# ConsenSys/gnark-crypto

Measured on NVIDIA H100. Metric: bn254 G1 MultiExp scalar-muls/s, higher is better.
Workload: dtype u32

## Files before the change

### gnark-crypto_b200/csrc/curve.cuh

```cuda
#pragma once
#include "field.cuh"
#include "fp2.cuh"

namespace gmsm {

template <class F>
struct Affine {
  F x, y;
  GMSM_HD bool is_inf() const { return x.is_zero() && y.is_zero(); }
  GMSM_HD static Affine inf() { return Affine{F::zero(), F::zero()}; }
};

template <class F>
struct XYZZ {
  F x, y, zz, zzz;
  GMSM_HD bool is_inf() const { return zz.is_zero(); }
  GMSM_HD static XYZZ inf() { return XYZZ{F::zero(), F::zero(), F::zero(), F::zero()}; }
};

template <class F>
struct Jac {
  F x, y, z;
};

template <class F>
GMSM_HD XYZZ<F> xyzz_from_affine(const Affine<F>& a) {
  if (a.is_inf()) return XYZZ<F>::inf();
  return XYZZ<F>{a.x, a.y, F::one(), F::one()};
}

template <class F>
GMSM_HD XYZZ<F> xyzz_double_affine(const F& x, const F& y) {
  F U = f_dbl(y);
  F V = f_sqr(U);
  F W = f_mul(U, V);
  F S = f_mul(x, V);
  F XX = f_sqr(x);
  F M = f_add(f_dbl(XX), XX);
  F S2 = f_dbl(S);
#if defined(GMSM_DOT2)
  XYZZ<F> r;
  r.x = f_sub(f_sqr(M), S2);
  r.y = f_dot2(f_sub(S, r.x), M, W, f_neg(y));
#else
  F L = f_mul(W, y);
  XYZZ<F> r;
  r.x = f_sub(f_sqr(M), S2);
  r.y = f_sub(f_mul(f_sub(S, r.x), M), L);
#endif
  r.zz = V;
  r.zzz = W;
  return r;
}

template <class F>
GMSM_HD void xyzz_add_mixed(XYZZ<F>& p, const Affine<F>& a, bool negate) {
  if (a.is_inf()) return;
  F ay = negate ? f_neg(a.y) : a.y;
  if (p.zz.is_zero()) {
    p.x = a.x;
    p.y = ay;
    p.zz = F::one();
    p.zzz = F::one();
    return;
  }
  F P = f_sub(f_mul(a.x, p.zz), p.x);
  F R = f_sub(f_mul(ay, p.zzz), p.y);
  if (P.is_zero()) {
    if (R.is_zero()) {
      p = xyzz_double_affine(a.x, ay);
    } else {
      p.zz = F::zero();
      p.zzz = F::zero();
    }
    return;
  }
  F PP = f_sqr(P);
  F PPP = f_mul(P, PP);
  F Q = f_mul(p.x, PP);
  F RR = f_sqr(R);
  F X3 = f_sub(f_sub(RR, PPP), f_dbl(Q));
#if defined(GMSM_DOT2)
  F Y3 = f_dot2(f_sub(Q, X3), R, f_neg(p.y), PPP);
#else
  F Y3 = f_sub(f_mul(f_sub(Q, X3), R), f_mul(p.y, PPP));
#endif
  p.x = X3;
  p.y = Y3;
  p.zz = f_mul(p.zz, PP);
  p.zzz = f_mul(p.zzz, PPP);
}

template <class F>
GMSM_HD XYZZ<F> xyzz_double(const XYZZ<F>& q) {
  F U = f_dbl(q.y);
  F V = f_sqr(U);
  F W = f_mul(U, V);
  F S = f_mul(q.x, V);
  F XX = f_sqr(q.x);
  F M = f_add(f_dbl(XX), XX);
  F U2 = f_mul(W, q.y);
  XYZZ<F> r;
  r.x = f_sub(f_sub(f_sqr(M), S), S);
  r.y = f_sub(f_mul(f_sub(S, r.x), M), U2);
  r.zz = f_mul(V, q.zz);
  r.zzz = f_mul(W, q.zzz);
  return r;
}

template <class F>
GMSM_HD void xyzz_add(XYZZ<F>& p, const XYZZ<F>& q) {
  if (q.zz.is_zero()) return;
  if (p.zz.is_zero()) {
    p = q;
    return;
  }
  F U2 = f_mul(q.x, p.zz);
  F U1 = f_mul(p.x, q.zz);
  F S2 = f_mul(q.y, p.zzz);
  F S1 = f_mul(p.y, q.zzz);
  F P = f_sub(U2, U1);
  F R = f_sub(S2, S1);
  if (P.is_zero()) {
    if (R.is_zero()) {
      p = xyzz_double(q);
    } else {
      p.zz = F::zero();
      p.zzz = F::zero();
    }
    return;
  }
  F PP = f_sqr(P);
  F PPP = f_mul(P, PP);
  F Q = f_mul(U1, PP);
#if defined(GMSM_DOT2)
  F X3 = f_sub(f_sub(f_sub(f_sqr(R), PPP), Q), Q);
  F Y3 = f_dot2(f_sub(Q, X3), R, f_neg(S1), PPP);
#else
  F V = f_mul(S1, PPP);
  F X3 = f_sub(f_sub(f_sub(f_sqr(R), PPP), Q), Q);
  F Y3 = f_sub(f_mul(f_sub(Q, X3), R), V);
#endif
  p.x = X3;
  p.y = Y3;
  p.zz = f_mul(f_mul(p.zz, q.zz), PP);
  p.zzz = f_mul(f_mul(p.zzz, q.zzz), PPP);
}

template <class F>
GMSM_HD Jac<F> jac_double(const Jac<F>& p) {
  F A = f_sqr(p.x);
  F B = f_sqr(p.y);
  F C = f_sqr(B);
  F D = f_sub(f_sub(f_sqr(f_add(p.x, B)), A), C);
  D = f_dbl(D);
  F E = f_add(f_dbl(A), A);
  F Fq = f_sqr(E);
  Jac<F> r;
  r.z = f_dbl(f_mul(p.y, p.z));
  r.x = f_sub(Fq, f_dbl(D));
  F C8 = f_dbl(f_dbl(f_dbl(C)));
  r.y = f_sub(f_mul(E, f_sub(D, r.x)), C8);
  return r;
}

static constexpr int TAB_M = 8;
template <class F, class Ld, class St, class Dbl>
GMSM_HD void table_level_batch(int cnt, int c, Ld ld, St st, Dbl dbl) {
  Jac<F> pts[TAB_M];
  F pref[TAB_M];
  F prod = F::one();
  for (int i = 0; i < cnt; i++) {
    const Affine<F> a = ld(i);
    Jac<F> j = a.is_inf() ? Jac<F>{F::zero(), F::zero(), F::zero()} : Jac<F>{a.x, a.y, F::one()};
    for (int l = 0; l < c; l++) j = dbl(j);
    pts[i] = j;
    pref[i] = prod;
    if (!j.z.is_zero()) prod = f_mul(prod, j.z);
  }
  F inv = f_inv(prod);
  for (int i = cnt - 1; i >= 0; i--) {
    Affine<F> a = Affine<F>::inf();
    if (!pts[i].z.is_zero()) {
      const F zi = f_mul(inv, pref[i]);
      inv = f_mul(inv, pts[i].z);
      const F z2 = f_sqr(zi);
      a.x = f_mul(pts[i].x, z2);
      a.y = f_mul(f_mul(pts[i].y, z2), zi);
    }
    st(i, a);
  }
}

template <class F>
GMSM_HD XYZZ<F> jac_to_xyzz(const Jac<F>& p) {
  XYZZ<F> r;
  r.x = p.x;
  r.y = p.y;
  r.zz = f_sqr(p.z);
  r.zzz = f_mul(r.zz, p.z);
  return r;
}

template <class F>
GMSM_HD Jac<F> xyzz_to_jac(const XYZZ<F>& p) {
  if (p.zz.is_zero()) return Jac<F>{F::zero(), F::zero(), F::zero()};
  Jac<F> j;
  j.x = f_mul(f_sqr(p.zz), p.x);
  j.y = f_mul(f_sqr(p.zzz), p.y);
  j.z = p.zzz;
  return j;
}

template <class F>
GMSM_HD Affine<F> jac_to_affine(const Jac<F>& j) {
  if (j.z.is_zero()) return Affine<F>::inf();
  F a = f_inv(j.z);
  F b = f_sqr(a);
  Affine<F> r;
  r.x = f_mul(j.x, b);
  r.y = f_mul(f_mul(j.y, b), a);
  return r;
}

}
```

### gnark-crypto_b200/csrc/field.cuh

```cuda
#pragma once
#include <cstdint>

#include "field_consts.cuh"
#include "hd.cuh"

namespace gmsm {

#if defined(GMSM_EMULATE_PTX) && !defined(__CUDACC__)
static thread_local uint32_t emu_cf = 0;
GMSM_D uint32_t emu_add(uint32_t a, uint32_t b, uint32_t cin, bool set) {
  uint64_t s = (uint64_t)a + b + cin;
  if (set) emu_cf = (uint32_t)(s >> 32);
  return (uint32_t)s;
}
GMSM_D uint32_t emu_sub(uint32_t a, uint32_t b, uint32_t bin, bool set) {
  uint64_t d = (uint64_t)a - b - bin;
  if (set) emu_cf = (uint32_t)(d >> 32) & 1;
  return (uint32_t)d;
}
GMSM_D uint32_t add_cc(uint32_t a, uint32_t b) { return emu_add(a, b, 0, true); }
GMSM_D uint32_t addc_cc(uint32_t a, uint32_t b) { return emu_add(a, b, emu_cf, true); }
GMSM_D uint32_t addc(uint32_t a, uint32_t b) { return emu_add(a, b, emu_cf, false); }
GMSM_D uint32_t sub_cc(uint32_t a, uint32_t b) { return emu_sub(a, b, 0, true); }
GMSM_D uint32_t subc_cc(uint32_t a, uint32_t b) { return emu_sub(a, b, emu_cf, true); }
// ... 48 lines not shown
GMSM_D uint32_t madc_hi_cc(uint32_t a, uint32_t b, uint32_t c) {
  uint32_t r;
  asm volatile("madc.hi.cc.u32 %0, %1, %2, %3;" : "=r"(r) : "r"(a), "r"(b), "r"(c));
  return r;
}
GMSM_D uint32_t madc_hi(uint32_t a, uint32_t b, uint32_t c) {
  uint32_t r;
  asm volatile("madc.hi.u32 %0, %1, %2, %3;" : "=r"(r) : "r"(a), "r"(b), "r"(c));
  return r;
}
#endif

template <class P>
struct Fp {
  static constexpr int N = P::N;
  using Params = P;
  uint32_t l[N];

  GMSM_HD static Fp zero() {
    Fp r;
#pragma unroll
    for (int i = 0; i < N; i++) r.l[i] = 0;
    return r;
  }
  GMSM_HD static Fp one() {
    Fp r;
#pragma unroll
    for (int i = 0; i < N; i++) r.l[i] = P::one(i);
    return r;
  }
  GMSM_HD bool is_zero() const {
    uint32_t o = 0;
#pragma unroll
    for (int i = 0; i < N; i++) o |= l[i];
    return o == 0;
  }
  GMSM_HD bool operator==(const Fp& b) const {
    uint32_t o = 0;
#pragma unroll
    for (int i = 0; i < N; i++) o |= l[i] ^ b.l[i];
    return o == 0;
  }
  GMSM_HD bool operator!=(const Fp& b) const { return !(*this == b); }
};

template <class P>
GMSM_HD uint32_t invm() {
#if defined(__CUDA_ARCH__)
  if constexpr (P::MOD_IN_CONST_BANK) return P::mod_cb(P::N);
  else
#endif
  return P::INV;
}
template <class P>
GMSM_HD uint32_t modm(int j) {
#if defined(__CUDA_ARCH__)
  if constexpr (P::MOD_IN_CONST_BANK) return P::mod_cb(j);
  else
#endif
  return P::mod(j);
}

template <class P>
GMSM_HD void fp_reduce_once(Fp<P>& a, uint32_t carry = 0) {
  constexpr int N = P::N;
  uint32_t t[N];
#if defined(GMSM_PTX_PATH)
  t[0] = sub_cc(a.l[0], P::mod(0));
#pragma unroll
  for (int i = 1; i < N; i++) t[i] = subc_cc(a.l[i], P::mod(i));
  uint32_t borrow = subc(0, 0);
  if constexpr (P::FULL) borrow = carry ? 0u : borrow;
#pragma unroll
  for (int i = 0; i < N; i++) a.l[i] = borrow ? a.l[i] : t[i];
#else
  uint64_t br = 0;
  for (int i = 0; i < N; i++) {
    uint64_t d = (uint64_t)a.l[i] - P::mod(i) - br;
    t[i] = (uint32_t)d;
    br = (d >> 32) & 1;
  }
  if (!br || carry)
    for (int i = 0; i < N; i++) a.l[i] = t[i];
#endif
}

template <class P>
GMSM_HD Fp<P> fp_add(const Fp<P>& a, const Fp<P>& b) {
  constexpr int N = P::N;
  Fp<P> r;
#if defined(GMSM_PTX_PATH)
  uint32_t c = 0;
  r.l[0] = add_cc(a.l[0], b.l[0]);
#pragma unroll
  for (int i = 1; i < N - 1; i++) r.l[i] = addc_cc(a.l[i], b.l[i]);
  if constexpr (P::FULL) {
    r.l[N - 1] = addc_cc(a.l[N - 1], b.l[N - 1]);
    c = addc(0, 0);
  } else {
    r.l[N - 1] = addc(a.l[N - 1], b.l[N - 1]);
  }
#else
  uint64_t c = 0;
  for (int i = 0; i < N; i++) {
    c += (uint64_t)a.l[i] + b.l[i];
    r.l[i] = (uint32_t)c;
    c >>= 32;
  }
#endif
  fp_reduce_once(r, (uint32_t)c);
  return r;
}

template <class P>
GMSM_HD Fp<P> fp_dbl(const Fp<P>& a) {
  return fp_add(a, a);
}

template <class P>
GMSM_HD Fp<P> fp_sub(const Fp<P>& a, const Fp<P>& b) {
  constexpr int N = P::N;
  Fp<P> r;
#if defined(GMSM_PTX_PATH)
  r.l[0] = sub_cc(a.l[0], b.l[0]);
#pragma unroll
  for (int i = 1; i < N; i++) r.l[i] = subc_cc(a.l[i], b.l[i]);
  uint32_t mask = subc(0, 0);
  r.l[0] = add_cc(r.l[0], P::mod(0) & mask);
#pragma unroll
  for (int i = 1; i < N - 1; i++) r.l[i] = addc_cc(r.l[i], P::mod(i) & mask);
  r.l[N - 1] = addc(r.l[N - 1], P::mod(N - 1) & mask);
#else
  uint64_t br = 0;
  for (int i = 0; i < N; i++) {
    uint64_t d = (uint64_t)a.l[i] - b.l[i] - br;
    r.l[i] = (uint32_t)d;
    br = (d >> 32) & 1;
  }
  if (br) {
    uint64_t c = 0;
    for (int i = 0; i < N; i++) {
      c += (uint64_t)r.l[i] + P::mod(i);
      r.l[i] = (uint32_t)c;
      c >>= 32;
    }
  }
#endif
  return r;
}

template <class P>
GMSM_HD Fp<P> fp_neg(const Fp<P>& a) {
  return fp_sub(Fp<P>::zero(), a);
}

template <class P>
GMSM_HD Fp<P> fp_mul_cios(const Fp<P>& x, const Fp<P>& y) {
  constexpr int N = P::N;
  Fp<P> r;
  uint32_t t[N + 2];
#pragma unroll
  for (int i = 0; i < N + 2; i++) t[i] = 0;
#pragma unroll
  for (int i = 0; i < N; i++) {
    uint64_t c = 0;
#pragma unroll
    for (int j = 0; j < N; j++) {
      c += (uint64_t)x.l[j] * y.l[i] + t[j];
      t[j] = (uint32_t)c;
      c >>= 32;
    }
    c += t[N];
    t[N] = (uint32_t)c;
    t[N + 1] = (uint32_t)(c >> 32);
    uint32_t m = t[0] * P::INV;
    c = (uint64_t)m * P::mod(0) + t[0];
    c >>= 32;
#pragma unroll
    for (int j = 1; j < N; j++) {
      c += (uint64_t)m * P::mod(j) + t[j];
      t[j - 1] = (uint32_t)c;
      c >>= 32;
    }
    c += t[N];
    t[N - 1] = (uint32_t)c;
    t[N] = t[N + 1] + (uint32_t)(c >> 32);
  }
#pragma unroll
  for (int i = 0; i < N; i++) r.l[i] = t[i];
  fp_reduce_once(r, t[N]);
  return r;
}

template <class P>
GMSM_HD Fp<P> fp_mul_inline(const Fp<P>& x, const Fp<P>& y) {
  constexpr int N = P::N;
  Fp<P> r;
#if defined(GMSM_PTX_PATH) && !defined(GMSM_PORTABLE_MUL)
  uint32_t A[N + 2], B[N + 2];
#pragma unroll
  for (int i = 0; i < N + 2; i++) A[i] = B[i] = 0;
  uint32_t dprev = 0;
  uint32_t e0prev = 0;
#pragma unroll
  for (int i = 0; i < N; i++) {
    uint32_t* Ev = (i & 1) ? B : A;
    uint32_t* Od = (i & 1) ? A : B;
    const uint32_t bi = y.l[i];
    const uint32_t d = (i == 0) ? 0u : Od[1];
    if (i == 0) {
      Ev[0] = mad_lo_cc(x.l[0], bi, Ev[0]);
    } else {
      (void)add_cc(e0prev, dprev);
      Ev[0] = madc_lo_cc(x.l[0], bi, Ev[0]);
    }
    Ev[1] = madc_hi_cc(x.l[0], bi, Ev[1]);
#pragma unroll
    for (int j = 2; j < N; j += 2) {
      Ev[j] = madc_lo_cc(x.l[j], bi, Ev[j]);
      Ev[j + 1] = madc_hi_cc(x.l[j], bi, Ev[j + 1]);
    }
    if constexpr (P::FULL) Ev[N] = addc(Ev[N], 0);
    else Ev[N] = addc(0, 0);
    Od[0] = mad_lo_cc(x.l[1], bi, Od[2]);
    Od[1] = madc_hi_cc(x.l[1], bi, Od[3]);
#pragma unroll
    for (int j = 2; j < N; j += 2) {
      Od[j] = madc_lo_cc(x.l[j + 1], bi, Od[j + 2]);
      Od[j + 1] = madc_hi_cc(x.l[j + 1], bi, Od[j + 3]);
    }
    Od[N] = 0;
    const uint32_t m = (Ev[0] + d) * invm<P>();
    Ev[0] = mad_lo_cc(modm<P>(0), m, Ev[0]);
    Ev[1] = madc_hi_cc(modm<P>(0), m, Ev[1]);
#pragma unroll
    for (int j = 2; j < N; j += 2) {
      Ev[j] = madc_lo_cc(modm<P>(j), m, Ev[j]);
      Ev[j + 1] = madc_hi_cc(modm<P>(j), m, Ev[j + 1]);
    }
    Ev[N] = addc(Ev[N], 0);
    Od[0] = mad_lo_cc(modm<P>(1), m, Od[0]);
    Od[1] = madc_hi_cc(modm<P>(1), m, Od[1]);
#pragma unroll
    for (int j = 2; j < N; j += 2) {
      Od[j] = madc_lo_cc(modm<P>(j + 1), m, Od[j]);
      Od[j + 1] = madc_hi_cc(modm<P>(j + 1), m, Od[j + 1]);
    }
    if constexpr (P::FULL) Od[N] = addc(0, 0);
    e0prev = Ev[0];
    dprev = d;
  }
  (void)add_cc(e0prev, dprev);
  r.l[0] = addc_cc(A[0], B[1]);
#pragma unroll
  for (int i = 1; i < N - 1; i++) r.l[i] = addc_cc(A[i], B[i + 1]);
  if constexpr (P::FULL) {
    r.l[N - 1] = addc_cc(A[N - 1], B[N]);
    fp_reduce_once(r, addc(A[N], 0));
  } else {
    r.l[N - 1] = addc(A[N - 1], B[N]);
    fp_reduce_once(r);
  }
#else
  return fp_mul_cios(x, y);
#endif
  return r;
}

#if defined(__CUDA_ARCH__) && defined(GMSM_MUL_NOINLINE)
template <class P> GMSM_HD Fp<P> fp_mul_karatsuba(const Fp<P>& x, const Fp<P>& y);
template <class P>
__device__ __noinline__ Fp<P> fp_mul_ni(Fp<P> x, Fp<P> y) {
#if defined(GMSM_MUL_KARATSUBA)
  if constexpr (P::N % 4 == 0 && (P::mod(P::N - 1) >> 30) == 0) return fp_mul_karatsuba(x, y);
  else
#endif
  return fp_mul_inline(x, y);
}
template <class P>
GMSM_HD Fp<P> fp_mul(const Fp<P>& x, const Fp<P>& y) {
  return fp_mul_ni<P>(x, y);
}
#else
template <class P> GMSM_HD Fp<P> fp_mul_karatsuba(const Fp<P>& x, const Fp<P>& y);
template <class P>
GMSM_HD Fp<P> fp_mul(const Fp<P>& x, const Fp<P>& y) {
#if defined(GMSM_MUL_KARATSUBA)
  if constexpr (P::N % 4 == 0 && (P::mod(P::N - 1) >> 30) == 0) return fp_mul_karatsuba(x, y);
  else
#endif
  return fp_mul_inline(x, y);
}
#endif

#if defined(GMSM_SQR_DEDICATED) && defined(GMSM_PTX_PATH) && !defined(GMSM_PORTABLE_MUL)
template <class P>
GMSM_HD Fp<P> fp_sqr_inline(const Fp<P>& x) {
  constexpr int N = P::N;
  static_assert((P::mod(N - 1) >> 30) == 0, "needs two spare top bits (2x in N limbs, frames below 3q)");
  Fp<P> r;
  uint32_t x2[N];
  x2[0] = x.l[0] << 1;
#pragma unroll
  for (int j = 1; j < N; j++) x2[j] = (x.l[j] << 1) | (x.l[j - 1] >> 31);
  uint32_t A[N + 2], B[N + 2];
#pragma unroll
// ... 449 lines not shown
      Ev[j] = madc_lo_cc(modm<P>(j), m, Ev[j]);
      Ev[j + 1] = madc_hi_cc(modm<P>(j), m, Ev[j + 1]);
    }
    Ev[N] = addc(Ev[N], 0);
    Od[0] = mad_lo_cc(modm<P>(1), m, Od[0]);
    Od[1] = madc_hi_cc(modm<P>(1), m, Od[1]);
#pragma unroll
    for (int j = 2; j < N; j += 2) {
      Od[j] = madc_lo_cc(modm<P>(j + 1), m, Od[j]);
      Od[j + 1] = madc_hi_cc(modm<P>(j + 1), m, Od[j + 1]);
    }
    GMSM_NO_CARRY();
    e0prev = Ev[0];
    dprev = d;
  }
  (void)add_cc(e0prev, dprev);
  out[0] = addc_cc(A[0], B[1]);
#pragma unroll
  for (int i = 1; i < N - 1; i++) out[i] = addc_cc(A[i], B[i + 1]);
  out[N - 1] = addc(A[N - 1], B[N]);
#else
  uint32_t t[N + 2];
  for (int i = 0; i < N; i++) t[i] = v[i];
  t[N] = t[N + 1] = 0;
  for (int i = 0; i < N; i++) {
    const uint32_t m = t[0] * P::INV;
    uint64_t c = (uint64_t)m * P::mod(0) + t[0];
    c >>= 32;
    for (int j = 1; j < N; j++) {
      c += (uint64_t)m * P::mod(j) + t[j];
      t[j - 1] = (uint32_t)c;
      c >>= 32;
    }
    c += t[N];
    t[N - 1] = (uint32_t)c;
    t[N] = (uint32_t)(c >> 32);
  }
  for (int i = 0; i < N; i++) out[i] = t[i];
#endif
}

template <class P, int NRED = 3>
GMSM_HD Fp<P> fp_redc_wide(const uint32_t* t) {
  constexpr int N = P::N;
  uint32_t lo[N];
  fp_redc_half<P>(t, lo);
  Fp<P> r;
#if defined(GMSM_PTX_PATH)
  r.l[0] = add_cc(lo[0], t[N]);
#pragma unroll
  for (int i = 1; i < N - 1; i++) r.l[i] = addc_cc(lo[i], t[N + i]);
  r.l[N - 1] = addc(lo[N - 1], t[2 * N - 1]);
#else
  uint64_t c = 0;
  for (int i = 0; i < N; i++) {
    c += (uint64_t)lo[i] + t[N + i];
    r.l[i] = (uint32_t)c;
    c >>= 32;
  }
#endif
#pragma unroll
  for (int k = 0; k < NRED; k++) fp_reduce_once(r);
  return r;
}

template <class P>
GMSM_HD Fp<P> fp_mul_karatsuba(const Fp<P>& x, const Fp<P>& y) {
  uint32_t t[2 * P::N];
  mul_wide_karatsuba<P::N>(x.l, y.l, t);
  return fp_redc_wide<P, 1>(t);
}

template <class P>
GMSM_HD Fp<P> fp_mul_split(const Fp<P>& x, const Fp<P>& y) {
  uint32_t t[2 * P::N];
  fp_mul_wide<P>(x.l, y.l, t);
  return fp_redc_wide<P>(t);
}

template <class P>
GMSM_HD Fp<P> fp_from_mont(const Fp<P>& x) {
  Fp<P> o = Fp<P>::zero();
  o.l[0] = 1;
  return fp_mul(x, o);
}

template <class P>
GMSM_HD Fp<P> fp_to_mont(const Fp<P>& x) {
  Fp<P> r2;
#pragma unroll
  for (int i = 0; i < P::N; i++) r2.l[i] = P::r2(i);
  return fp_mul(x, r2);
}

template <class P>
GMSM_HD Fp<P> fp_inv_fermat(const Fp<P>& x) {
  constexpr int N = P::N;
  uint32_t e[N];
  {
    uint64_t br = 2;
    for (int i = 0; i < N; i++) {
      uint64_t d = (uint64_t)P::mod(i) - br;
      e[i] = (uint32_t)d;
      br = (d >> 32) & 1;
    }
  }
  Fp<P> acc = Fp<P>::one();
  bool started = false;
  for (int i = 32 * N - 1; i >= 0; i--) {
    if (started) acc = fp_sqr(acc);
    if ((e[i >> 5] >> (i & 31)) & 1) {
      acc = started ? fp_mul(acc, x) : x;
      started = true;
    }
  }
  return acc;
}

template <class P>
GMSM_HD Fp<P> fp_inv(const Fp<P>& x) {
  constexpr int N = P::N;
  if (x.is_zero()) return x;
  uint32_t u[N], v[N], x1[N], x2[N];
  for (int i = 0; i < N; i++) { u[i] = x.l[i]; v[i] = P::mod(i); x1[i] = 0; x2[i] = 0; }
  x1[0] = 1;
  auto is_one = [](const uint32_t* a) { uint32_t o = a[0] ^ 1u; for (int i = 1; i < N; i++) o |= a[i]; return o == 0; };
  auto shr1 = [](uint32_t* a, uint32_t top) { for (int i = 0; i < N - 1; i++) a[i] = (a[i] >> 1) | (a[i + 1] << 31); a[N - 1] = (a[N - 1] >> 1) | (top << 31); };
  auto add_mod = [](uint32_t* a) { uint64_t c = 0; for (int i = 0; i < N; i++) { c += (uint64_t)a[i] + P::mod(i); a[i] = (uint32_t)c; c >>= 32; } return (uint32_t)c; };
  auto geq = [](const uint32_t* a, const uint32_t* b) { for (int i = N - 1; i >= 0; i--) { if (a[i] != b[i]) return a[i] > b[i]; } return true; };
  auto sub = [](uint32_t* a, const uint32_t* b) { uint64_t br = 0; for (int i = 0; i < N; i++) { uint64_t d = (uint64_t)a[i] - b[i] - br; a[i] = (uint32_t)d; br = (d >> 32) & 1; } return (uint32_t)br; };
  auto halve = [&](uint32_t* w, uint32_t* y) {
    shr1(w, 0);
    const uint32_t top = (y[0] & 1u) ? add_mod(y) : 0u;
    shr1(y, top);
  };
  auto sub_mod = [&](uint32_t* a, const uint32_t* b) { if (sub(a, b)) add_mod(a); };
  while (!is_one(u) && !is_one(v)) {
    while (!(u[0] & 1u)) halve(u, x1);
    while (!(v[0] & 1u)) halve(v, x2);
    if (geq(u, v)) { sub(u, v); sub_mod(x1, x2); } else { sub(v, u); sub_mod(x2, x1); }
  }
  Fp<P> r, r2;
  for (int i = 0; i < N; i++) { r.l[i] = is_one(u) ? x1[i] : x2[i]; r2.l[i] = P::r2(i); }
  return fp_mul(fp_mul(r, r2), r2);
}

template <class P> GMSM_HD Fp<P> f_add(const Fp<P>& a, const Fp<P>& b) { return fp_add(a, b); }
template <class P> GMSM_HD Fp<P> f_sub(const Fp<P>& a, const Fp<P>& b) { return fp_sub(a, b); }
template <class P> GMSM_HD Fp<P> f_mul(const Fp<P>& a, const Fp<P>& b) { return fp_mul(a, b); }
template <class P> GMSM_HD Fp<P> f_sqr(const Fp<P>& a) { return fp_sqr(a); }
template <class P> GMSM_HD Fp<P> f_dot2(const Fp<P>& x, const Fp<P>& y, const Fp<P>& u, const Fp<P>& v) { return fp_dot2(x, y, u, v); }
template <class P> GMSM_HD Fp<P> f_dbl(const Fp<P>& a) { return fp_dbl(a); }
template <class P> GMSM_HD Fp<P> f_neg(const Fp<P>& a) { return fp_neg(a); }
template <class P> GMSM_HD Fp<P> f_inv(const Fp<P>& a) { return fp_inv(a); }

}
```

### gnark-crypto_b200/csrc/fp2.cuh

```cuda
#pragma once
#include "field.cuh"

namespace gmsm {

template <class P>
struct Fp2 {
  using Params = P;
  static constexpr int N = 2 * P::N;
  Fp<P> a0, a1;
  GMSM_HD static Fp2 zero() { return Fp2{Fp<P>::zero(), Fp<P>::zero()}; }
  GMSM_HD static Fp2 one() { return Fp2{Fp<P>::one(), Fp<P>::zero()}; }
  GMSM_HD bool is_zero() const { return a0.is_zero() && a1.is_zero(); }
  GMSM_HD bool operator==(const Fp2& b) const { return a0 == b.a0 && a1 == b.a1; }
  GMSM_HD bool operator!=(const Fp2& b) const { return !(*this == b); }
};

template <class P> GMSM_HD Fp2<P> f_add(const Fp2<P>& a, const Fp2<P>& b) { return Fp2<P>{fp_add(a.a0, b.a0), fp_add(a.a1, b.a1)}; }
template <class P> GMSM_HD Fp2<P> f_sub(const Fp2<P>& a, const Fp2<P>& b) { return Fp2<P>{fp_sub(a.a0, b.a0), fp_sub(a.a1, b.a1)}; }
template <class P> GMSM_HD Fp2<P> f_dbl(const Fp2<P>& a) { return Fp2<P>{fp_dbl(a.a0), fp_dbl(a.a1)}; }
template <class P> GMSM_HD Fp2<P> f_neg(const Fp2<P>& a) { return Fp2<P>{fp_neg(a.a0), fp_neg(a.a1)}; }

template <class P>
GMSM_HD Fp<P> fp_mul_by5(const Fp<P>& c) {
  return fp_add(fp_dbl(fp_dbl(c)), c);
}

#if defined(GMSM_FP2_LAZY)
template <class P>
GMSM_HD Fp2<P> fp2_mul_lazy_inline(const Fp2<P>& x, const Fp2<P>& y) {
    constexpr int N = P::N;
    uint32_t sx[N], sy[N], T0[2 * N], T1[2 * N], T2[2 * N];
#if defined(GMSM_PTX_PATH)
    sx[0] = add_cc(x.a0.l[0], x.a1.l[0]);
#pragma unroll
    for (int i = 1; i < N - 1; i++) sx[i] = addc_cc(x.a0.l[i], x.a1.l[i]);
    sx[N - 1] = addc(x.a0.l[N - 1], x.a1.l[N - 1]);
    sy[0] = add_cc(y.a0.l[0], y.a1.l[0]);
#pragma unroll
    for (int i = 1; i < N - 1; i++) sy[i] = addc_cc(y.a0.l[i], y.a1.l[i]);
    sy[N - 1] = addc(y.a0.l[N - 1], y.a1.l[N - 1]);
#else
    { uint64_t c = 0; for (int i = 0; i < N; i++) { c += (uint64_t)x.a0.l[i] + x.a1.l[i]; sx[i] = (uint32_t)c; c >>= 32; } }
    { uint64_t c = 0; for (int i = 0; i < N; i++) { c += (uint64_t)y.a0.l[i] + y.a1.l[i]; sy[i] = (uint32_t)c; c >>= 32; } }
#endif
    fp_mul_wide<P>(x.a0.l, y.a0.l, T0);
    fp_mul_wide<P>(x.a1.l, y.a1.l, T1);
    fp_mul_wide<P>(sx, sy, T2);
#if defined(GMSM_PTX_PATH)
    T2[0] = sub_cc(T2[0], T0[0]);
#pragma unroll
    for (int i = 1; i < 2 * N - 1; i++) T2[i] = subc_cc(T2[i], T0[i]);
    T2[2 * N - 1] = subc(T2[2 * N - 1], T0[2 * N - 1]);
    T2[0] = sub_cc(T2[0], T1[0]);
#pragma unroll
    for (int i = 1; i < 2 * N - 1; i++) T2[i] = subc_cc(T2[i], T1[i]);
    T2[2 * N - 1] = subc(T2[2 * N - 1], T1[2 * N - 1]);
    T0[0] = sub_cc(T0[0], T1[0]);
#pragma unroll
    for (int i = 1; i < 2 * N - 1; i++) T0[i] = subc_cc(T0[i], T1[i]);
    T0[2 * N - 1] = subc(T0[2 * N - 1], T1[2 * N - 1]);
    T0[N] = add_cc(T0[N], P::mod(0));
#pragma unroll
    for (int i = 1; i < N - 1; i++) T0[N + i] = addc_cc(T0[N + i], P::mod(i));
    T0[2 * N - 1] = addc(T0[2 * N - 1], P::mod(N - 1));
#else
    { uint64_t br = 0; for (int i = 0; i < 2 * N; i++) { uint64_t d = (uint64_t)T2[i] - T0[i] - br; T2[i] = (uint32_t)d; br = (d >> 32) & 1; } }
    { uint64_t br = 0; for (int i = 0; i < 2 * N; i++) { uint64_t d = (uint64_t)T2[i] - T1[i] - br; T2[i] = (uint32_t)d; br = (d >> 32) & 1; } }
    { uint64_t br = 0; for (int i = 0; i < 2 * N; i++) { uint64_t d = (uint64_t)T0[i] - T1[i] - br; T0[i] = (uint32_t)d; br = (d >> 32) & 1; } }
    { uint64_t c = 0; for (int i = 0; i < N; i++) { c += (uint64_t)T0[N + i] + P::mod(i); T0[N + i] = (uint32_t)c; c >>= 32; } }
#endif
    Fp2<P> z;
    z.a1 = fp_redc_wide<P, 1>(T2);
    z.a0 = fp_redc_wide<P, 2>(T0);
    return z;
}
#if defined(__CUDA_ARCH__) && defined(GMSM_MUL_NOINLINE)
template <class P>
__device__ __noinline__ Fp2<P> fp2_mul_lazy_ni(Fp2<P> x, Fp2<P> y) {
  return fp2_mul_lazy_inline(x, y);
}
#endif
#endif

template <class P>
GMSM_HD Fp2<P> f_mul(const Fp2<P>& x, const Fp2<P>& y) {
  static_assert(P::FP2_NONRES == -1 || P::FP2_NONRES == -5, "supported quadratic non-residues");
#if defined(GMSM_FP2_LAZY)
  if constexpr (P::FP2_NONRES == -1 && (P::mod(P::N - 1) >> 30) == 0) {
#if defined(__CUDA_ARCH__) && defined(GMSM_MUL_NOINLINE)
    return fp2_mul_lazy_ni<P>(x, y);
#else
    return fp2_mul_lazy_inline(x, y);
#endif
  }
#endif
#if defined(GMSM_FP2_DOT2) && defined(GMSM_DOT2)
  Fp2<P> z;
  const Fp<P> by1 = (P::FP2_NONRES == -5) ? fp_neg(fp_mul_by5(y.a1)) : fp_neg(y.a1);
  z.a0 = fp_dot2(x.a0, y.a0, x.a1, by1);
  z.a1 = fp_dot2(x.a0, y.a1, x.a1, y.a0);
  return z;
#else
  Fp<P> a = fp_add(x.a0, x.a1);
  Fp<P> b = fp_add(y.a0, y.a1);
  a = fp_mul(a, b);
  b = fp_mul(x.a0, y.a0);
  Fp<P> c = fp_mul(x.a1, y.a1);
  Fp2<P> z;
  z.a1 = fp_sub(fp_sub(a, b), c);
  if (P::FP2_NONRES == -5) c = fp_mul_by5(c);
  z.a0 = fp_sub(b, c);
  return z;
#endif
}

template <class P>
GMSM_HD Fp2<P> f_sqr(const Fp2<P>& x) {
  Fp<P> a = fp_add(x.a0, x.a1);
  Fp<P> b = (P::FP2_NONRES == -5) ? fp_sub(x.a0, fp_mul_by5(x.a1)) : fp_sub(x.a0, x.a1);
  a = fp_mul(a, b);
  b = fp_dbl(fp_mul(x.a0, x.a1));
  if (P::FP2_NONRES == -5) a = fp_add(a, fp_dbl(b));
  return Fp2<P>{a, b};
}

template <class P>
GMSM_HD Fp2<P> f_dot2(const Fp2<P>& x, const Fp2<P>& y, const Fp2<P>& u, const Fp2<P>& v) {
#if defined(GMSM_DOT4)
  const Fp<P> by1 = (P::FP2_NONRES == -5) ? fp_neg(fp_mul_by5(y.a1)) : fp_neg(y.a1);
  const Fp<P> bv1 = (P::FP2_NONRES == -5) ? fp_neg(fp_mul_by5(v.a1)) : fp_neg(v.a1);
  Fp2<P> z;
  z.a0 = fp_dot4(x.a0, y.a0, x.a1, by1, u.a0, v.a0, u.a1, bv1);
  z.a1 = fp_dot4(x.a0, y.a1, x.a1, y.a0, u.a0, v.a1, u.a1, v.a0);
  return z;
#else
  return f_add(f_mul(x, y), f_mul(u, v));
#endif
}

template <class P>
GMSM_HD Fp2<P> f_inv(const Fp2<P>& x) {
  Fp<P> t0 = fp_sqr(x.a0);
  Fp<P> t1 = fp_sqr(x.a1);
  if (P::FP2_NONRES == -5) t1 = fp_mul_by5(t1);
  t0 = fp_add(t0, t1);
  t1 = fp_inv(t0);
  return Fp2<P>{fp_mul(x.a0, t1), fp_neg(fp_mul(x.a1, t1))};
}

}
```

### gnark-crypto_b200/csrc/testops.cuh

```cuda
#pragma once
#include "groups.cuh"

namespace gmsm {

template <class T>
GMSM_HD T rd(const uint32_t* p) {
  T r;
  uint32_t* w = reinterpret_cast<uint32_t*>(&r);
  for (int i = 0; i < (int)(sizeof(T) / 4); i++) w[i] = p[i];
  return r;
}
template <class T>
GMSM_HD void wr(uint32_t* p, const T& r) {
  const uint32_t* w = reinterpret_cast<const uint32_t*>(&r);
  for (int i = 0; i < (int)(sizeof(T) / 4); i++) p[i] = w[i];
}

template <class G>
GMSM_HD void test_op_sizes(int op, int* wa, int* wb, int* wo) {
  constexpr int FW = G::F::N;
  switch (op) {
    case 0: case 1: case 2: *wa = FW; *wb = FW; *wo = FW; break;
    case 3: case 4: case 5: case 6: *wa = FW; *wb = 0; *wo = FW; break;
    case 7: case 8: *wa = 4 * FW; *wb = 2 * FW; *wo = 4 * FW; break;
    case 9: *wa = 4 * FW; *wb = 4 * FW; *wo = 4 * FW; break;
    case 10: *wa = 4 * FW; *wb = 0; *wo = 4 * FW; break;
    case 11: *wa = 4 * FW; *wb = 0; *wo = 2 * FW; break;
    case 12: *wa = G::Fr::N; *wb = 0; *wo = G::Fr::N; break;
    case 13: *wa = 2 * FW; *wb = 2 * FW; *wo = FW; break;
    default: *wa = *wb = *wo = 0;
  }
}

template <class G>
GMSM_HD void test_op_one(int op, const uint32_t* a, const uint32_t* b, uint32_t* o) {
  using F = typename G::F;
  switch (op) {
    case 0: wr(o, f_mul(rd<F>(a), rd<F>(b))); break;
    case 1: wr(o, f_add(rd<F>(a), rd<F>(b))); break;
    case 2: wr(o, f_sub(rd<F>(a), rd<F>(b))); break;
    case 3: wr(o, f_sqr(rd<F>(a))); break;
    case 4: wr(o, f_neg(rd<F>(a))); break;
    case 5: wr(o, f_dbl(rd<F>(a))); break;
    case 6: wr(o, f_inv(rd<F>(a))); break;
    case 7: case 8: {
      XYZZ<F> p = rd<XYZZ<F>>(a);
      xyzz_add_mixed(p, rd<Affine<F>>(b), op == 8);
      wr(o, p);
    } break;
    case 9: {
      XYZZ<F> p = rd<XYZZ<F>>(a);
      xyzz_add(p, rd<XYZZ<F>>(b));
      wr(o, p);
    } break;
    case 10: wr(o, xyzz_double(rd<XYZZ<F>>(a))); break;
    case 11: wr(o, jac_to_affine(xyzz_to_jac(rd<XYZZ<F>>(a)))); break;
    case 12: wr(o, fp_from_mont(rd<typename G::Fr>(a))); break;
    case 13: wr(o, f_dot2(rd<F>(a), rd<F>(b), rd<F>(a + G::F::N), rd<F>(b + G::F::N))); break;
    default: break;
  }
}


}
```

### include/gmsm.h

```cpp
#ifndef GMSM_H
#define GMSM_H

#include <stddef.h>
#include <stdint.h>

#ifdef __cplusplus
extern "C" {
#endif

typedef enum {
  GMSM_BN254_G1 = 0,
  GMSM_BN254_G2 = 1,
  GMSM_BLS12381_G1 = 2,
  GMSM_BLS12381_G2 = 3,
  GMSM_BLS12377_G1 = 4,
  GMSM_BLS12377_G2 = 5,
  GMSM_SECP256K1_G1 = 6,
  GMSM_BW6761_G1 = 7,
  GMSM_BW6761_G2 = 8,
  GMSM_BLS24315_G1 = 9,
  GMSM_BLS24317_G1 = 10,
  GMSM_BW6633_G1 = 11,
  GMSM_BW6633_G2 = 12
} gmsm_curve_t;

enum {
  GMSM_OK = 0,
  GMSM_EINVAL = 1,
  GMSM_ECUDA = 2,
  GMSM_ENOMEM = 3,
  GMSM_ENODEV = 4
};

const char* gmsm_last_error(void);
const char* gmsm_version(void);

size_t gmsm_affine_bytes(gmsm_curve_t curve);
size_t gmsm_scalar_bytes(gmsm_curve_t curve);
size_t gmsm_jac_bytes(gmsm_curve_t curve);
size_t gmsm_xyzz_bytes(gmsm_curve_t curve);

int gmsm_bn254_g1_multiexp(const uint64_t* points, const uint64_t* scalars, size_t n, int nb_tasks,
                           uint64_t out_jac[12]);
int gmsm_bn254_g2_multiexp(const uint64_t* points, const uint64_t* scalars, size_t n, int nb_tasks,
                           uint64_t out_jac[24]);
int gmsm_bls12381_g1_multiexp(const uint64_t* points, const uint64_t* scalars, size_t n, int nb_tasks,
                              uint64_t out_jac[18]);
int gmsm_bls12381_g2_multiexp(const uint64_t* points, const uint64_t* scalars, size_t n, int nb_tasks,
                              uint64_t out_jac[36]);
int gmsm_bls12377_g1_multiexp(const uint64_t* points, const uint64_t* scalars, size_t n, int nb_tasks,
                              uint64_t out_jac[18]);
int gmsm_bls12377_g2_multiexp(const uint64_t* points, const uint64_t* scalars, size_t n, int nb_tasks,
                              uint64_t out_jac[36]);
int gmsm_secp256k1_g1_multiexp(const uint64_t* points, const uint64_t* scalars, size_t n, int nb_tasks,
                               uint64_t out_jac[12]);
int gmsm_bw6761_g1_multiexp(const uint64_t* points, const uint64_t* scalars , size_t n, int nb_tasks,
                            uint64_t out_jac[36]);
int gmsm_bw6761_g2_multiexp(const uint64_t* points, const uint64_t* scalars , size_t n, int nb_tasks,
                            uint64_t out_jac[36]);
int gmsm_bls24315_g1_multiexp(const uint64_t* points, const uint64_t* scalars, size_t n, int nb_tasks,
                              uint64_t out_jac[15]);
int gmsm_bls24317_g1_multiexp(const uint64_t* points, const uint64_t* scalars, size_t n, int nb_tasks,
                              uint64_t out_jac[15]);
int gmsm_bw6633_g1_multiexp(const uint64_t* points, const uint64_t* scalars , size_t n, int nb_tasks,
                            uint64_t out_jac[30]);
int gmsm_bw6633_g2_multiexp(const uint64_t* points, const uint64_t* scalars , size_t n, int nb_tasks,
                            uint64_t out_jac[30]);
int gmsm_multiexp(gmsm_curve_t curve, const uint64_t* points, const uint64_t* scalars, size_t n,
                  int nb_tasks, uint64_t* out_jac);
int gmsm_choose_window_bits(gmsm_curve_t curve, size_t n_total);
int gmsm_multiexp_window_sums(gmsm_curve_t curve, const uint64_t* points, const uint64_t* scalars, size_t n, int c,
                              int device, void* out_partials);
int gmsm_last_oneshot_launches(void);

typedef struct gmsm_bases gmsm_bases_t;
gmsm_bases_t* gmsm_bases_upload(gmsm_curve_t curve, const uint64_t* points, size_t n, int device);
int gmsm_bases_multiexp(gmsm_bases_t* bases, size_t offset, const uint64_t* scalars, size_t n,
                        int nb_tasks, uint64_t* out_jac);
void gmsm_bases_free(gmsm_bases_t* bases);
int gmsm_bases_multiexp_device(gmsm_bases_t* bases, size_t offset, const void* d_scalars, size_t n, int nb_tasks,
                               uint64_t* out_jac, void* stream);
int gmsm_bases_precompute(gmsm_bases_t* bases, int c);
int gmsm_bases_table_bits(const gmsm_bases_t* bases);

typedef struct gmsm_ctx gmsm_ctx_t;
gmsm_ctx_t* gmsm_ctx_create(gmsm_curve_t curve, size_t max_n, int c, int device);
void gmsm_ctx_destroy(gmsm_ctx_t* ctx);
int gmsm_ctx_window_bits(const gmsm_ctx_t* ctx);
int gmsm_ctx_num_windows(const gmsm_ctx_t* ctx);
size_t gmsm_ctx_workspace_bytes(const gmsm_ctx_t* ctx);
int gmsm_ctx_last_launches(const gmsm_ctx_t* ctx);
int gmsm_ctx_msm_device(gmsm_ctx_t* ctx, const void* d_points, const void* d_scalars, size_t n,
                        void* d_out_jac, void* stream);
int gmsm_ctx_window_sums_device(gmsm_ctx_t* ctx, const void* d_points, const void* d_scalars, size_t n,
                                void* d_partials, void* stream);
int gmsm_ctx_finalize_device(gmsm_ctx_t* ctx, const void* d_partials, int nranks, void* d_out_jac,
                             void* stream);
gmsm_ctx_t* gmsm_ctx_create_tables(gmsm_curve_t curve, size_t max_n, int c, int device);
int gmsm_tables_build_device(gmsm_curve_t curve, int c, const void* d_points, size_t n, void* d_table,
                             size_t row_stride, void* stream);
int gmsm_ctx_msm_tables_device(gmsm_ctx_t* ctx, const void* d_table, size_t row_stride, size_t offset,
                               const void* d_scalars, size_t n, void* d_out_jac, void* stream);
void gmsm_ctx_set_profiling(gmsm_ctx_t* ctx, int on);
int gmsm_ctx_last_stage_ms(gmsm_ctx_t* ctx, float out_ms[8]);

int gmsm_generate_multiples_device(gmsm_curve_t curve, const uint64_t* base_affine_host, uint64_t start,
                                   size_t n, void* d_out_points, void* stream);

int gmsm_batch_scalar_mul(gmsm_curve_t curve, const uint64_t* base_affine, const uint64_t* scalars, size_t n,
                          uint64_t* out_points);

int gmsm_g1_decode(gmsm_curve_t curve, const uint8_t* bytes, size_t n, int raw, int check_on_curve, uint64_t* out_points);
int gmsm_g1_decode_device(gmsm_curve_t curve, const void* d_bytes, size_t n, int raw, int check_on_curve, void* d_points,
                          void* d_first_error, void* stream);

typedef struct gmsm_fft_domain gmsm_fft_domain_t;
enum {
  GMSM_FR_BN254 = 0, GMSM_FR_BLS12381 = 1, GMSM_FR_BLS12377 = 2,
  GMSM_FR_BLS24315 = 3,
  GMSM_FR_BLS24317 = 4,
  GMSM_FR_BW6633 = 5,
  GMSM_FR_BW6761 = 6
};
enum { GMSM_DIT = 0, GMSM_DIF = 1 };
size_t gmsm_fft_fr_bytes(int fr_field);
gmsm_fft_domain_t* gmsm_fft_domain_create(int fr_field, uint64_t m, const uint64_t* shift, int device);
void gmsm_fft_domain_free(gmsm_fft_domain_t* domain);
uint64_t gmsm_fft_domain_cardinality(const gmsm_fft_domain_t* domain);
int gmsm_fft_domain_constants(const gmsm_fft_domain_t* domain, uint64_t* out);
int gmsm_fft(gmsm_fft_domain_t* domain, uint64_t* a, size_t n, int decimation, int coset);
int gmsm_fft_inverse(gmsm_fft_domain_t* domain, uint64_t* a, size_t n, int decimation, int coset);
int gmsm_fft_device(gmsm_fft_domain_t* domain, void* d_a, size_t n, int inverse, int decimation, int coset, void* stream);
int gmsm_fft_bit_reverse_device(gmsm_fft_domain_t* domain, void* d_a, size_t n, void* stream);

size_t gmsm_fr_poly_workspace_bytes(int fr_field, size_t n);
int gmsm_fr_poly_div_x_minus_a_device(int fr_field, const void* d_f, size_t n, const uint64_t* a, void* d_h, void* d_fa,
                                      void* d_work, void* stream);
int gmsm_fr_poly_fold_device(int fr_field, const void* const* d_polys, const size_t* lens, size_t k, const uint64_t* gamma,
                             void* d_out, size_t out_len, void* stream);
int gmsm_fr_poly_lincomb_device(int fr_field, const void* const* d_polys, const size_t* lens, const uint64_t* scalars,
                                const size_t* strides, const size_t* offsets, size_t k, void* d_out, size_t out_len, int accumulate,
                                void* stream);

int gmsm_fr_batch_invert_device(int fr_field, const void* d_a, size_t n, void* d_out, void* stream);
size_t gmsm_fr_permutation_workspace_bytes(int fr_field, size_t n);
int gmsm_fr_permutation_accumulate_device(int fr_field, const void* d_t1, const void* d_t2, size_t n, const uint64_t* epsilon,
                                          void* d_z, void* d_work, void* stream);
int gmsm_fft_permutation_numerator_device(gmsm_fft_domain_t* domain, const void* d_lt1, const void* d_lt2, const void* d_lz, size_t n,
                                          const uint64_t* epsilon, const uint64_t* omega, void* d_out, void* stream);

size_t gmsm_g1_to_lagrange_workspace_bytes(gmsm_curve_t curve, size_t n);
int gmsm_g1_to_lagrange(gmsm_curve_t curve, const uint64_t* points, size_t n, int device, uint64_t* out);
int gmsm_g1_to_lagrange_device(gmsm_curve_t curve, const void* d_points, size_t n, void* d_out, void* d_work, void* stream);

enum {
  GMSM_OP_FMUL = 0, GMSM_OP_FADD = 1, GMSM_OP_FSUB = 2, GMSM_OP_FSQR = 3, GMSM_OP_FNEG = 4,
  GMSM_OP_FDBL = 5, GMSM_OP_FINV = 6,
  GMSM_OP_ADD_MIXED = 7,
  GMSM_OP_SUB_MIXED = 8,
  GMSM_OP_ADD = 9,
  GMSM_OP_DOUBLE = 10,
  GMSM_OP_TO_AFFINE = 11,
  GMSM_OP_FR_FROM_MONT = 12,
  GMSM_OP_FDOT2 = 13
};
int gmsm_test_op(gmsm_curve_t curve, int op, const uint32_t* a, const uint32_t* b, uint32_t* out,
                 size_t n);
int gmsm_test_digits(gmsm_curve_t curve, int c, const uint64_t* scalars, size_t n, uint32_t* out);

#ifdef __cplusplus
}
#endif
#endif
```

Measured before the change: 300.8 million.

## Add FP64-FMA wide multiplier option and cheaper unreduced negation for products

Adds an optional Montgomery multiply and dot-product path for 8-limb fields. It splits operands into 52-bit limbs held in doubles, forms the partial products with FMA-based exact splitting, accumulates them as integer bit patterns, then normalises and reduces. Each multiply site in mixed addition can be switched to this path through a compile-time mask, which defaults to off. Independently, negations that only feed a multiply now use a plain p−a with no conditional correction. That saves a little integer work on the default path, but it relies on multiplies accepting an operand equal to p.

```diff
diff --git a/gnark-crypto_b200/csrc/curve.cuh b/gnark-crypto_b200/csrc/curve.cuh
--- a/gnark-crypto_b200/csrc/curve.cuh
+++ b/gnark-crypto_b200/csrc/curve.cuh
@@ -1,4 +1,7 @@
 #pragma once
+#include <type_traits>
+
+#include "f64mul.cuh"
 #include "field.cuh"
 #include "fp2.cuh"
 
@@ -41,7 +44,7 @@
 #if defined(GMSM_DOT2)
   XYZZ<F> r;
   r.x = f_sub(f_sqr(M), S2);
-  r.y = f_dot2(f_sub(S, r.x), M, W, f_neg(y));
+  r.y = f_dot2(f_sub(S, r.x), M, W, f_neg_operand(y));
 #else
   F L = f_mul(W, y);
   XYZZ<F> r;
@@ -53,42 +56,67 @@
   return r;
 }
 
+#ifndef GMSM_F64_MASK
+#define GMSM_F64_MASK 0
+#endif
+template <int BIT, class F>
+GMSM_HD constexpr bool f64_product() {
+  if constexpr (((GMSM_F64_MASK >> BIT) & 1) && std::is_same<F, Fp<typename F::Params>>::value) {
+    if constexpr (F::N == 8) return (F::Params::mod(7) >> 30) == 0;
+  }
+  return false;
+}
+template <int BIT, class F>
+GMSM_HD F h_mul(const F& x, const F& y) {
+  if constexpr (f64_product<BIT, F>()) return fp_mul_f64(x, y);
+  else return f_mul(x, y);
+}
+template <int BIT, class F>
+GMSM_HD F h_sqr(const F& x) {
+  if constexpr (f64_product<BIT, F>()) return fp_mul_f64(x, x);
+  else return f_sqr(x);
+}
+template <int BIT, class F>
+GMSM_HD F h_dot2(const F& x, const F& y, const F& u, const F& v) {
+  if constexpr (f64_product<BIT, F>()) return fp_dot2_f64(x, y, u, v);
+  else return f_dot2(x, y, u, v);
+}
+
 template <class F>
 GMSM_HD void xyzz_add_mixed(XYZZ<F>& p, const Affine<F>& a, bool negate) {
   if (a.is_inf()) return;
-  F ay = negate ? f_neg(a.y) : a.y;
   if (p.zz.is_zero()) {
     p.x = a.x;
-    p.y = ay;
+    p.y = negate ? f_neg(a.y) : a.y;
     p.zz = F::one();
     p.zzz = F::one();
     return;
   }
-  F P = f_sub(f_mul(a.x, p.zz), p.x);
-  F R = f_sub(f_mul(ay, p.zzz), p.y);
+  F P = f_sub(h_mul<0>(a.x, p.zz), p.x);
+  F R = f_sub(h_mul<1>(negate ? f_neg_operand(a.y) : a.y, p.zzz), p.y);
   if (P.is_zero()) {
     if (R.is_zero()) {
-      p = xyzz_double_affine(a.x, ay);
+      p = xyzz_double_affine(a.x, negate ? f_neg(a.y) : a.y);
     } else {
       p.zz = F::zero();
       p.zzz = F::zero();
     }
     return;
   }
-  F PP = f_sqr(P);
-  F PPP = f_mul(P, PP);
-  F Q = f_mul(p.x, PP);
-  F RR = f_sqr(R);
+  F PP = h_sqr<2>(P);
+  F PPP = h_mul<3>(P, PP);
+  F Q = h_mul<4>(p.x, PP);
+  F RR = h_sqr<5>(R);
   F X3 = f_sub(f_sub(RR, PPP), f_dbl(Q));
 #if defined(GMSM_DOT2)
-  F Y3 = f_dot2(f_sub(Q, X3), R, f_neg(p.y), PPP);
+  F Y3 = h_dot2<6>(f_sub(Q, X3), R, f_neg_operand(p.y), PPP);
 #else
   F Y3 = f_sub(f_mul(f_sub(Q, X3), R), f_mul(p.y, PPP));
 #endif
   p.x = X3;
   p.y = Y3;
-  p.zz = f_mul(p.zz, PP);
-  p.zzz = f_mul(p.zzz, PPP);
+  p.zz = h_mul<7>(p.zz, PP);
+  p.zzz = h_mul<8>(p.zzz, PPP);
 }
 
 template <class F>
@@ -135,7 +163,7 @@
   F Q = f_mul(U1, PP);
 #if defined(GMSM_DOT2)
   F X3 = f_sub(f_sub(f_sub(f_sqr(R), PPP), Q), Q);
-  F Y3 = f_dot2(f_sub(Q, X3), R, f_neg(S1), PPP);
+  F Y3 = f_dot2(f_sub(Q, X3), R, f_neg_operand(S1), PPP);
 #else
   F V = f_mul(S1, PPP);
   F X3 = f_sub(f_sub(f_sub(f_sqr(R), PPP), Q), Q);
diff --git a/gnark-crypto_b200/csrc/f64mul.cuh b/gnark-crypto_b200/csrc/f64mul.cuh
--- /dev/null
+++ b/gnark-crypto_b200/csrc/f64mul.cuh
@@ -0,0 +1,164 @@
+#pragma once
+#include <cstdint>
+#if !defined(__CUDA_ARCH__)
+#include <cmath>
+#include <cstring>
+#endif
+
+#include "field.cuh"
+
+namespace gmsm {
+
+GMSM_HD double f64_fma(double a, double b, double c) {
+#if defined(__CUDA_ARCH__)
+  return __fma_rn(a, b, c);
+#else
+  return std::fma(a, b, c);
+#endif
+}
+GMSM_HD double f64_add(double a, double b) {
+#if defined(__CUDA_ARCH__)
+  return __dadd_rn(a, b);
+#else
+  return a + b;
+#endif
+}
+GMSM_HD uint64_t f64_bits(double d) {
+#if defined(__CUDA_ARCH__)
+  return (uint64_t)__double_as_longlong(d);
+#else
+  uint64_t u;
+  std::memcpy(&u, &d, 8);
+  return u;
+#endif
+}
+GMSM_HD double f64_from_words(uint32_t hi, uint32_t lo) {
+#if defined(__CUDA_ARCH__)
+  return __hiloint2double((int)hi, (int)lo);
+#else
+  const uint64_t u = ((uint64_t)hi << 32) | lo;
+  double d;
+  std::memcpy(&d, &u, 8);
+  return d;
+#endif
+}
+
+constexpr int F64_LIMBS = 5;
+constexpr int F64_COLS = 10;
+
+GMSM_HD uint32_t f64_bits_at(const uint32_t* x, int o) {
+  const int w = o >> 5, s = o & 31;
+  const uint32_t lo = w < 8 ? x[w] : 0u, hi = w + 1 < 8 ? x[w + 1] : 0u;
+  return s ? (lo >> s) | (hi << (32 - s)) : lo;
+}
+
+GMSM_HD void f64_split(const uint32_t* x, double* a) {
+#pragma unroll
+  for (int k = 0; k < F64_LIMBS; k++) {
+    const uint32_t lo = f64_bits_at(x, 52 * k), hi = f64_bits_at(x, 52 * k + 32) & 0xfffffu;
+    a[k] = f64_add(f64_from_words(0x43300000u | hi, lo), -0x1p52);
+  }
+}
+
+template <int NP>
+GMSM_HD constexpr uint64_t f64_col_const(int c) {
+  constexpr uint64_t KH = 0x4670000000000000ull;
+  constexpr uint64_t KL = 0x4338000000000000ull;
+  auto terms = [](int col) { return (col < 0 || col > 8) ? 0 : (col <= 4 ? col + 1 : 9 - col); };
+  uint64_t k = 0;
+  k -= (uint64_t)(NP * terms(c)) * KL;
+  k -= (uint64_t)(NP * terms(c - 1)) * KH;
+  if (c <= 8) k += 1ull << 57;
+  if (c >= 1) k -= 32;
+  return k;
+}
+
+GMSM_HD void f64_accumulate(const double* a, const double* b, uint64_t* S) {
+#pragma unroll
+  for (int i = 0; i < F64_LIMBS; i++) {
+#pragma unroll
+    for (int j = 0; j < F64_LIMBS; j++) {
+      const double h = f64_fma(a[i], b[j], 0x1p104);
+      const double t = f64_add(h, -0x1p104);
+      const double l = f64_fma(a[i], b[j], -t);
+      const double lb = f64_add(l, 0x1.8p52);
+      S[i + j] += f64_bits(lb);
+      S[i + j + 1] += f64_bits(h);
+    }
+  }
+}
+
+GMSM_HD void f64_normalize(const uint64_t* S, uint32_t* t) {
+  uint32_t E[16], O[16];
+#pragma unroll
+  for (int i = 0; i < 16; i++) E[i] = O[i] = 0;
+#pragma unroll
+  for (int c = 0; c < F64_COLS; c++) {
+    uint32_t* W = (c & 1) ? O : E;
+    const int w = (52 * c) >> 5, s = (52 * c) & 31;
+    const uint32_t lo = (uint32_t)S[c], hi = (uint32_t)(S[c] >> 32);
+    if (s == 0) {
+      W[w] = lo;
+      if (w + 1 < 16) W[w + 1] = hi;
+    } else {
+      W[w] = lo << s;
+      if (w + 1 < 16) W[w + 1] = (lo >> (32 - s)) | (hi << s);
+      if (w + 2 < 16) W[w + 2] = hi >> (32 - s);
+    }
+  }
+#if defined(GMSM_PTX_PATH)
+  t[0] = add_cc(E[0], O[0]);
+#pragma unroll
+  for (int i = 1; i < 15; i++) t[i] = addc_cc(E[i], O[i]);
+  t[15] = addc(E[15], O[15]);
+#else
+  uint64_t c = 0;
+  for (int i = 0; i < 16; i++) {
+    c += (uint64_t)E[i] + O[i];
+    t[i] = (uint32_t)c;
+    c >>= 32;
+  }
+#endif
+}
+
+GMSM_HD void f64_mul_wide(const uint32_t* x, const uint32_t* y, uint32_t* t) {
+  double a[F64_LIMBS], b[F64_LIMBS];
+  f64_split(x, a);
+  f64_split(y, b);
+  uint64_t S[F64_COLS];
+#pragma unroll
+  for (int c = 0; c < F64_COLS; c++) S[c] = f64_col_const<1>(c);
+  f64_accumulate(a, b, S);
+  f64_normalize(S, t);
+}
+
+GMSM_HD void f64_dot2_wide(const uint32_t* x, const uint32_t* y, const uint32_t* u, const uint32_t* v, uint32_t* t) {
+  double a[F64_LIMBS], b[F64_LIMBS];
+  uint64_t S[F64_COLS];
+#pragma unroll
+  for (int c = 0; c < F64_COLS; c++) S[c] = f64_col_const<2>(c);
+  f64_split(x, a);
+  f64_split(y, b);
+  f64_accumulate(a, b, S);
+  f64_split(u, a);
+  f64_split(v, b);
+  f64_accumulate(a, b, S);
+  f64_normalize(S, t);
+}
+
+template <class P>
+GMSM_HD Fp<P> fp_mul_f64(const Fp<P>& x, const Fp<P>& y) {
+  static_assert(P::N == 8 && (P::mod(P::N - 1) >> 30) == 0, "8 limbs, two spare top bits");
+  uint32_t t[16];
+  f64_mul_wide(x.l, y.l, t);
+  return fp_redc_wide<P, 1>(t);
+}
+template <class P>
+GMSM_HD Fp<P> fp_dot2_f64(const Fp<P>& x, const Fp<P>& y, const Fp<P>& u, const Fp<P>& v) {
+  static_assert(P::N == 8 && (P::mod(P::N - 1) >> 30) == 0, "8 limbs, two spare top bits");
+  uint32_t t[16];
+  f64_dot2_wide(x.l, y.l, u.l, v.l, t);
+  return fp_redc_wide<P, 2>(t);
+}
+
+}
diff --git a/gnark-crypto_b200/csrc/field.cuh b/gnark-crypto_b200/csrc/field.cuh
--- a/gnark-crypto_b200/csrc/field.cuh
+++ b/gnark-crypto_b200/csrc/field.cuh
@@ -224,6 +224,26 @@
 template <class P>
 GMSM_HD Fp<P> fp_neg(const Fp<P>& a) {
   return fp_sub(Fp<P>::zero(), a);
+}
+
+template <class P>
+GMSM_HD Fp<P> fp_neg_operand(const Fp<P>& a) {
+  constexpr int N = P::N;
+  Fp<P> r;
+#if defined(GMSM_PTX_PATH)
+  r.l[0] = sub_cc(P::mod(0), a.l[0]);
+#pragma unroll
+  for (int i = 1; i < N - 1; i++) r.l[i] = subc_cc(P::mod(i), a.l[i]);
+  r.l[N - 1] = subc(P::mod(N - 1), a.l[N - 1]);
+#else
+  uint64_t br = 0;
+  for (int i = 0; i < N; i++) {
+    uint64_t d = (uint64_t)P::mod(i) - a.l[i] - br;
+    r.l[i] = (uint32_t)d;
+    br = (d >> 32) & 1;
+  }
+#endif
+  return r;
 }
 
 template <class P>
@@ -979,6 +999,7 @@
 template <class P> GMSM_HD Fp<P> f_dot2(const Fp<P>& x, const Fp<P>& y, const Fp<P>& u, const Fp<P>& v) { return fp_dot2(x, y, u, v); }
 template <class P> GMSM_HD Fp<P> f_dbl(const Fp<P>& a) { return fp_dbl(a); }
 template <class P> GMSM_HD Fp<P> f_neg(const Fp<P>& a) { return fp_neg(a); }
+template <class P> GMSM_HD Fp<P> f_neg_operand(const Fp<P>& a) { return fp_neg_operand(a); }
 template <class P> GMSM_HD Fp<P> f_inv(const Fp<P>& a) { return fp_inv(a); }
 
 }
diff --git a/gnark-crypto_b200/csrc/fp2.cuh b/gnark-crypto_b200/csrc/fp2.cuh
--- a/gnark-crypto_b200/csrc/fp2.cuh
+++ b/gnark-crypto_b200/csrc/fp2.cuh
@@ -19,6 +19,7 @@
 template <class P> GMSM_HD Fp2<P> f_sub(const Fp2<P>& a, const Fp2<P>& b) { return Fp2<P>{fp_sub(a.a0, b.a0), fp_sub(a.a1, b.a1)}; }
 template <class P> GMSM_HD Fp2<P> f_dbl(const Fp2<P>& a) { return Fp2<P>{fp_dbl(a.a0), fp_dbl(a.a1)}; }
 template <class P> GMSM_HD Fp2<P> f_neg(const Fp2<P>& a) { return Fp2<P>{fp_neg(a.a0), fp_neg(a.a1)}; }
+template <class P> GMSM_HD Fp2<P> f_neg_operand(const Fp2<P>& a) { return f_neg(a); }
 
 template <class P>
 GMSM_HD Fp<P> fp_mul_by5(const Fp<P>& c) {
diff --git a/gnark-crypto_b200/csrc/testops.cuh b/gnark-crypto_b200/csrc/testops.cuh
--- a/gnark-crypto_b200/csrc/testops.cuh
+++ b/gnark-crypto_b200/csrc/testops.cuh
@@ -28,6 +28,10 @@
     case 11: *wa = 4 * FW; *wb = 0; *wo = 2 * FW; break;
     case 12: *wa = G::Fr::N; *wb = 0; *wo = G::Fr::N; break;
     case 13: *wa = 2 * FW; *wb = 2 * FW; *wo = FW; break;
+    case 14:
+      if (std::is_same<typename G::F, Fp<typename G::F::Params>>::value && FW == 8) { *wa = 2 * FW; *wb = 2 * FW; *wo = 8 * FW; }
+      else *wa = *wb = *wo = 0;
+      break;
     default: *wa = *wb = *wo = 0;
   }
 }
@@ -57,6 +61,21 @@
     case 11: wr(o, jac_to_affine(xyzz_to_jac(rd<XYZZ<F>>(a)))); break;
     case 12: wr(o, fp_from_mont(rd<typename G::Fr>(a))); break;
     case 13: wr(o, f_dot2(rd<F>(a), rd<F>(b), rd<F>(a + G::F::N), rd<F>(b + G::F::N))); break;
+    case 14:
+      if constexpr (std::is_same<F, Fp<typename F::Params>>::value && F::N == 8) {
+        uint32_t t2[16];
+        f64_mul_wide(a, b, o);
+        mul_wide_limbs<8>(a, b, o + 16);
+        f64_dot2_wide(a, b, a + 8, b + 8, o + 32);
+        mul_wide_limbs<8>(a + 8, b + 8, t2);
+        uint64_t c = 0;
+        for (int i = 0; i < 16; i++) {
+          c += (uint64_t)o[16 + i] + t2[i];
+          o[48 + i] = (uint32_t)c;
+          c >>= 32;
+        }
+      }
+      break;
     default: break;
   }
 }
diff --git a/include/gmsm.h b/include/gmsm.h
--- a/include/gmsm.h
+++ b/include/gmsm.h
@@ -162,7 +162,8 @@
   GMSM_OP_DOUBLE = 10,
   GMSM_OP_TO_AFFINE = 11,
   GMSM_OP_FR_FROM_MONT = 12,
-  GMSM_OP_FDOT2 = 13
+  GMSM_OP_FDOT2 = 13,
+  GMSM_OP_F64_WIDE = 14
 };
 int gmsm_test_op(gmsm_curve_t curve, int op, const uint32_t* a, const uint32_t* b, uint32_t* out,
                  size_t n);
```

New measurement: 306.7 million (median of 6 runs). 2.0% higher.
